# apache/arrow

Hardware: AMD Instinct MI355X
Metric: filter_take_mrows_per_s (higher is better)
Workload: dtype int64; 1 GPU; Filter+Take int64[1000000000] + validity (10% null), boolean mask 10% true, FilterOptions::DROP; take indices = the mask's row numbers (monotonic; indices_nonzero: uint64 through CallFunction, GetTakeIndices: uint32 in the mirror), no boundscheck; inputs = splitmix64 streams of SURVEY.md 8(d) (seeds 1,2,3); rows=1000000000, selected_rows=99992053, parallelism=single-gpu

## Files before the change

### arrow_amd/csrc/selection.hip

```cpp
#include "arx_common.h"

#include <string.h>

#include <algorithm>
#include <type_traits>

namespace arx {

struct FilterWsHeader {
  int64_t total;
  int64_t ntiles;
  int64_t ngroups;
  int64_t length;
  int64_t valid;
  int64_t pad[3];
};
static_assert(sizeof(FilterWsHeader) == 64, "header is one 64-byte line");

struct FilterWsView {
  FilterWsHeader* hdr;
  int64_t* group_excl;
  int64_t* group_total;
  uint32_t* tile_counts;
  int64_t* group_valid;
};

static inline int64_t num_tiles(int64_t length) { return ceil_div(length, kTileRows); }
static inline int64_t num_groups(int64_t length) {
  return ceil_div(num_tiles(length), kTilesPerGroup);
}

static inline FilterWsView ws_view(void* ws, int64_t length) {
  FilterWsView v;
  const int64_t ng = num_groups(length);
  uint8_t* p = static_cast<uint8_t*>(ws);
  v.hdr = reinterpret_cast<FilterWsHeader*>(p);
  v.group_excl = reinterpret_cast<int64_t*>(p + 64);
  v.group_total = v.group_excl + ng;
  v.tile_counts = reinterpret_cast<uint32_t*>(v.group_total + ng);
  v.group_valid = reinterpret_cast<int64_t*>(v.tile_counts + ng * kTilesPerGroup);
  return v;
}

__device__ __forceinline__ uint64_t emit_word(const Bits& mask, const Bits& mvalid, int64_t w,
                                              bool emit_null, bool invert,
                                              uint64_t* mask_valid_out) {
  uint64_t m = load_word(mask, w);
  const uint64_t mv = load_word(mvalid, w);
  *mask_valid_out = mv;
  if (emit_null || invert) {
    const uint64_t in_range = load_word(Bits{nullptr, 0, mask.length, 0}, w);
    if (invert) m = ~m & in_range;
    if (emit_null) return (m | ~mv) & in_range;
  }
  return m & mv;
}

template <bool VALID>
__global__ __launch_bounds__(kBlock) void count_kernel(Bits mask, Bits mvalid, Bits vvalid, int emit_null,
                                                       int invert, int64_t ntiles,
                                                       uint32_t* tile_counts,
                                                       int64_t* group_total, int64_t* group_valid) {
  __shared__ uint32_t wave_sums[kWavesPerBlock];
  __shared__ uint32_t wave_valid[kWavesPerBlock];
  const int lane = lane_id();
  const int wave = threadIdx.x >> 6;
  const int64_t group = blockIdx.x;
  const int64_t t0 = group * kTilesPerGroup + wave * 16;
  uint32_t mine = 0;
  uint32_t kv = 0;
#pragma unroll 4
  for (int i = 0; i < 16; ++i) {
    const int64_t t = t0 + i;
    uint32_t k = 0;
    if (t < ntiles) {
      uint64_t mv;
      const uint64_t e = emit_word(mask, mvalid, t * 64 + lane, emit_null != 0, invert != 0, &mv);
      k = __popcll(e);
      if constexpr (VALID) kv += __popcll(e & mv & load_word(vvalid, t * 64 + lane));
    }
    const uint32_t s = wave_reduce_sum_u32(k);
    if (lane == i) mine = s;
  }
  if (lane < 16) tile_counts[t0 + lane] = mine;
  const uint32_t wsum = wave_reduce_sum_u32(lane < 16 ? mine : 0u);
  if (lane == 0) wave_sums[wave] = wsum;
  if constexpr (VALID) {
    const uint32_t vsum = wave_reduce_sum_u32(kv);
    if (lane == 0) wave_valid[wave] = vsum;
  }
  __syncthreads();
  if (threadIdx.x == 0) {
    int64_t s = 0, v = 0;
    for (int i = 0; i < kWavesPerBlock; ++i) {
      s += wave_sums[i];
      if constexpr (VALID) v += wave_valid[i];
    }
    group_total[group] = s;
    if constexpr (VALID) group_valid[group] = v;
  }
}

__global__ __launch_bounds__(1024) void scan_kernel(const int64_t* group_total, int64_t ngroups,
                                                    int64_t* group_excl, FilterWsHeader* hdr,
                                                    const int64_t* group_valid = nullptr) {
  __shared__ int64_t wave_tot[16];
  __shared__ int64_t carry_s;
  __shared__ unsigned long long valid_s;
  const int tid = threadIdx.x;
  const int lane = tid & 63;
  const int wave = tid >> 6;
  if (tid == 0) carry_s = 0;
  if (tid == 0) valid_s = 0;
  __syncthreads();
  if (group_valid != nullptr) {
    int64_t mine = 0;
    for (int64_t i = tid; i < ngroups; i += 1024) mine += group_valid[i];
#pragma unroll
    for (int d = 32; d >= 1; d >>= 1) mine += __shfl_xor(mine, d, 64);
    if (lane == 0 && mine != 0) atomicAdd(&valid_s, static_cast<unsigned long long>(mine));
    __syncthreads();
  }
  for (int64_t base = 0; base < ngroups; base += 1024) {
    const int64_t i = base + tid;
    const int64_t v = i < ngroups ? group_total[i] : 0;
    int64_t x = v;
#pragma unroll
    for (int d = 1; d < 64; d <<= 1) {
      const int64_t n = __shfl_up(x, d, 64);
      if (lane >= d) x += n;
    }
    if (lane == 63) wave_tot[wave] = x;
    __syncthreads();
    int64_t wave_prefix = 0;
    for (int k = 0; k < wave; ++k) wave_prefix += wave_tot[k];
    const int64_t carry = carry_s;
    if (i < ngroups) group_excl[i] = carry + wave_prefix + x - v;
    __syncthreads();
    if (tid == 1023) carry_s = carry + wave_prefix + x;
    __syncthreads();
  }
  if (tid == 0) {
    hdr->total = carry_s;
    hdr->valid = static_cast<int64_t>(valid_s);
  }
}

struct CompactArgs {
  const uint8_t* values;
  Bits mask;
  Bits mvalid;
  Bits vvalid;
  int64_t length;
  int64_t ntiles;
  const uint32_t* tile_counts;
  const int64_t* group_excl;
  uint8_t* out_data;
  uint64_t* out_validity;
  int emit_null;
  int invert;
  int values_aligned16;
};

constexpr int kFlushBytes = 2048;

template <int RING>
struct __attribute__((aligned(16))) CompactLds {
  uint8_t ring[kWavesPerBlock][RING];
  uint64_t vbits[kWavesPerBlock][72];
};

template <int W>
struct ElemT;
template <> struct ElemT<1> { using type = uint8_t; };
template <> struct ElemT<2> { using type = uint16_t; };
template <> struct ElemT<4> { using type = uint32_t; };
template <> struct ElemT<8> { using type = uint64_t; };
template <> struct ElemT<16> { using type = uint4; };
struct Elem32 { uint4 lo, hi; };
template <> struct ElemT<32> { using type = Elem32; };

template <int W>
__device__ __forceinline__ typename ElemT<W>::type zero_elem() {
  if constexpr (W == 32) {
    return Elem32{make_uint4(0, 0, 0, 0), make_uint4(0, 0, 0, 0)};
  } else if constexpr (W == 16) {
    return make_uint4(0, 0, 0, 0);
  } else {
    return 0;
  }
}

constexpr int kSelNt = 3;

template <int W>
__device__ __forceinline__ typename ElemT<W>::type sel_load(const typename ElemT<W>::type* p, bool nt) {
  using E = typename ElemT<W>::type;
  if constexpr (W == 32) {
    return *p;
  } else if constexpr (W == 16) {
    return nt ? nt_load16(p) : *p;
  } else {
    return nt ? nt_load<E>(p) : *p;
  }
}
template <int W>
__device__ __forceinline__ void sel_store(typename ElemT<W>::type* p, typename ElemT<W>::type v) {
  using E = typename ElemT<W>::type;
  if constexpr (W == 32) {
    *p = v;
  } else if constexpr (W == 16) {
    if constexpr ((kSelNt & 2) != 0) nt_store16(p, v); else *p = v;
  } else {
    if constexpr ((kSelNt & 2) != 0) nt_store<E>(p, v); else *p = v;
  }
}

__device__ __forceinline__ void wave_lds_sync() {
  __builtin_amdgcn_fence(__ATOMIC_RELEASE, "wavefront");
  __builtin_amdgcn_wave_barrier();
  __builtin_amdgcn_fence(__ATOMIC_ACQUIRE, "wavefront");
}

template <int W, int RING>
__device__ __forceinline__ void flush_region(const uint8_t* ring, uint8_t* gbase, int64_t F,
                                             int64_t lo, int64_t hi, int lane) {
  using E = typename ElemT<W>::type;
  constexpr int R = 16 / W;
  const int ring_off = static_cast<int>(F & (RING - 1));
#pragma unroll
  for (int h = 0; h < kFlushBytes / (16 * kWave); ++h) {
    const int g = h * kWave + lane;
    const int64_t gs = F + g * 16;
    const int64_t ge = gs + 16;
    if (ge <= lo || gs >= hi) continue;
    const uint8_t* src = ring + ring_off + g * 16;
    uint8_t* dst = gbase + gs;
    if (gs >= lo && ge <= hi) {
      sel_store<16>(reinterpret_cast<uint4*>(dst), *reinterpret_cast<const uint4*>(src));
    } else {
#pragma unroll
      for (int e = 0; e < R; ++e) {
        const int64_t es = gs + e * W;
        if (es >= lo && es + W <= hi) {
          *reinterpret_cast<E*>(dst + e * W) = *reinterpret_cast<const E*>(src + e * W);
        }
      }
    }
  }
}

template <int W, int B>
struct Batch {
  using E = typename ElemT<W>::type;
  static constexpr int R = 16 / W;
  uint32_t bits[B];
  uint32_t zbits[B];
  uint32_t rank[B];
  E v[B][R];
};

template <int R, bool EMIT>
__device__ __forceinline__ void select_words(uint64_t Ew, uint32_t p, uint64_t Zw,
                                             int widx_base, int lane, uint64_t* wE, uint32_t* wp,
                                             uint64_t* wZ) {
  constexpr int kLanesPerWord = 64 / R;
  const int q_mine = lane / kLanesPerWord;
  uint64_t e = 0, z = 0;
  uint32_t pp = 0;
#pragma unroll
  for (int q = 0; q < R; ++q) {
    const int src = widx_base + q;
    const uint32_t lo = __builtin_amdgcn_readlane(static_cast<uint32_t>(Ew), src);
    const uint32_t hi = __builtin_amdgcn_readlane(static_cast<uint32_t>(Ew >> 32), src);
    const uint32_t pq = __builtin_amdgcn_readlane(p, src);
    uint64_t zq = 0;
    if constexpr (EMIT) {
      const uint32_t zlo = __builtin_amdgcn_readlane(static_cast<uint32_t>(Zw), src);
      const uint32_t zhi = __builtin_amdgcn_readlane(static_cast<uint32_t>(Zw >> 32), src);
      zq = (static_cast<uint64_t>(zhi) << 32) | zlo;
    }
    if (q == q_mine) {
      e = (static_cast<uint64_t>(hi) << 32) | lo;
      pp = pq;
      z = zq;
    }
  }
  *wE = e;
  *wp = pp;
  *wZ = z;
}

struct TileCtx {
  uint64_t Ew, Zw;
  uint32_t p;
  int lane;
  int64_t tile_row0;
  const uint8_t* values;
  __amdgpu_buffer_rsrc_t rsrc;
};

template <int W, bool IOTA, bool EMIT, bool ALIGNED, int B>
__device__ __forceinline__ void issue_batch(const TileCtx& c, int j0, Batch<W, B>& b) {
  using E = typename ElemT<W>::type;
  constexpr int R = 16 / W;
  constexpr int kRowsPerIter = kWave * R;
#pragma unroll
  for (int i = 0; i < B; ++i) {
    const int j = j0 + i;
    const int row_in_tile = j * kRowsPerIter + c.lane * R;
    const int bpos = row_in_tile & 63;
    uint64_t wE, wZ;
    uint32_t wp;
    select_words<R, EMIT>(c.Ew, c.p, c.Zw, j * R, c.lane, &wE, &wp, &wZ);
    b.bits[i] = static_cast<uint32_t>(wE >> bpos) & ((1u << R) - 1u);
    b.zbits[i] = static_cast<uint32_t>(wZ >> bpos) & ((1u << R) - 1u);
    b.rank[i] = wp + __popcll(wE & low_mask64(bpos));
    if constexpr (IOTA) {
#pragma unroll
      for (int r = 0; r < R; ++r) b.v[i][r] = static_cast<E>(c.tile_row0 + row_in_tile + r);
    } else {
      const int64_t row = c.tile_row0 + row_in_tile;
      const uint8_t* src = c.values + row * static_cast<int64_t>(W);
      if constexpr (ALIGNED) {
        const uint32_t voff = b.bits[i] != 0 ? static_cast<uint32_t>(row_in_tile * W) : kBufferSkip;
        const uint4 q = (kSelNt & 1) ? buffer_load_b128_nt(c.rsrc, voff) : buffer_load_b128(c.rsrc, voff);
        if constexpr (W == 16) {
          b.v[i][0] = q;
        } else {
          const E* qe = reinterpret_cast<const E*>(&q);
#pragma unroll
          for (int r = 0; r < R; ++r) b.v[i][r] = qe[r];
        }
      } else {
#pragma unroll
        for (int r = 0; r < R; ++r) {
          b.v[i][r] = zero_elem<W>();
          if ((b.bits[i] >> r) & 1u) {
            if constexpr (W == 16) {
              const uint64_t* s64 = reinterpret_cast<const uint64_t*>(src + r * W);
              const uint64_t lo64 = s64[0], hi64 = s64[1];
              b.v[i][r] = make_uint4(static_cast<uint32_t>(lo64), static_cast<uint32_t>(lo64 >> 32),
                                     static_cast<uint32_t>(hi64), static_cast<uint32_t>(hi64 >> 32));
            } else {
              b.v[i][r] = *reinterpret_cast<const E*>(src + r * W);
            }
          }
        }
      }
    }
  }
}

template <int W, int B, int RING>
__device__ __forceinline__ void consume_batch(const Batch<W, B>& b, uint8_t* ring, int64_t a0) {
  using E = typename ElemT<W>::type;
  constexpr int R = 16 / W;
#pragma unroll
  for (int i = 0; i < B; ++i) {
    if (b.bits[i] != 0) {
      uint32_t rk = b.rank[i];
#pragma unroll
      for (int r = 0; r < R; ++r) {
        if ((b.bits[i] >> r) & 1u) {
          E e = b.v[i][r];
          if ((b.zbits[i] >> r) & 1u) e = zero_elem<W>();
          const int ro = static_cast<int>((a0 + static_cast<int64_t>(rk) * W) & (RING - 1));
          *reinterpret_cast<E*>(ring + ro) = e;
          ++rk;
        }
      }
    }
  }
}

template <int W, bool IOTA, bool EMIT, bool ALIGNED, int B, bool PIPE>
__global__ __launch_bounds__(kBlock) void compact_kernel(CompactArgs a) {
  using E = typename ElemT<W>::type;
  constexpr int R = 16 / W;
  constexpr int kRowsPerIter = kWave * R;
  constexpr int kIters = kTileRows / kRowsPerIter;
  constexpr int kWordsPerIter = kRowsPerIter / 64;
  constexpr int kBatches = kIters / B;
  constexpr int RING = (B <= 2) ? 4096 : 8192;
  static_assert(kIters % B == 0, "batch must divide the iteration count");
  static_assert(!PIPE || kBatches % 2 == 0, "pipelined form walks the batches in pairs");

  __shared__ CompactLds<RING> lds;

  const int lane = lane_id();
  const int wave = __builtin_amdgcn_readfirstlane(threadIdx.x >> 6);
  const int64_t t = static_cast<int64_t>(blockIdx.x) * kWavesPerBlock + wave;
  if (t >= a.ntiles) return;

  const int64_t w = t * 64 + lane;
  uint64_t mv;
  const uint64_t Ew = emit_word(a.mask, a.mvalid, w, EMIT, a.invert != 0, &mv);
  const uint32_t k = __popcll(Ew);
  const uint32_t incl = wave_inclusive_scan_u32(k);
  const uint32_t p = incl - k;
  const uint32_t total = __shfl(incl, 63, 64);
  if (total == 0) return;

  const int64_t grp = t >> 6;
  const int tin = static_cast<int>(t & 63);
  const uint32_t cprev = lane < tin ? a.tile_counts[grp * kTilesPerGroup + lane] : 0u;
  const int64_t off = a.group_excl[grp] + wave_reduce_sum_u32(cprev);

  uint8_t* ring = lds.ring[wave];
  const int64_t a0 =
      static_cast<int64_t>((reinterpret_cast<uint64_t>(a.out_data) + static_cast<uint64_t>(off) * W) &
                           (kFlushBytes - 1));
  uint8_t* gbase = a.out_data + (off * static_cast<int64_t>(W) - a0);
  int64_t flushed = 0;

  TileCtx c;
  c.Ew = Ew;
  c.Zw = EMIT ? (Ew & ~mv) : 0;
  c.p = p;
  c.lane = lane;
  c.tile_row0 = t * kTileRows;
  c.values = a.values;
  c.rsrc = make_rsrc(IOTA ? nullptr : a.values + c.tile_row0 * static_cast<int64_t>(W),
                     static_cast<uint32_t>(kTileRows * W));

  auto flush_check = [&](int next_batch) {
    const uint32_t cum = next_batch < kBatches
                             ? __builtin_amdgcn_readlane(p, next_batch * B * kWordsPerIter)
                             : total;
    const int64_t written = a0 + static_cast<int64_t>(cum) * W;
    if (written - flushed >= kFlushBytes) {
      wave_lds_sync();
      while (written - flushed >= kFlushBytes) {
        flush_region<W, RING>(ring, gbase, flushed, a0, written, lane);
        flushed += kFlushBytes;
      }
      wave_lds_sync();
    }
  };

  bool tile_done = false;
  if constexpr (IOTA) {
    if (a0 + static_cast<int64_t>(total) * W <= RING) {
      uint64_t m = Ew;
      uint32_t rk = p;
      while (m != 0) {
        const int bpos = __ffsll(static_cast<unsigned long long>(m)) - 1;
// ... 301 lines not shown
    const int64_t base = c * (64 * U);
    int64_t pos[U];
    uint64_t idx[U];
    bool ok[U];
#pragma unroll
    for (int u = 0; u < U; ++u) {
      const int64_t p = base + u * 64 + lane;
      pos[u] = p <= last ? p : last;
      idx[u] = static_cast<uint64_t>((kSelNt & 1) ? nt_load<IdxT>(indices + pos[u]) : indices[pos[u]]);
    }
#pragma unroll
    for (int u = 0; u < U; ++u) {
      ok[u] = (base + u * 64 + lane) <= last;
      if constexpr (HAS_IV) {
        const uint64_t wbits = load_word_nb(a.ivalid, (base >> 6) + u);
        ok[u] = ok[u] && ((wbits >> lane) & 1ull);
      }
    }
    E val[U];
#pragma unroll
    for (int u = 0; u < U; ++u) {
      const E* src = ok[u] ? (values + idx[u]) : (out + pos[u]);
      val[u] = sel_load<W>(src, (kSelNt & 4) != 0);
    }
    if constexpr (HAS_SV) {
      uint8_t vb[U];
#pragma unroll
      for (int u = 0; u < U; ++u) {
        const uint64_t bit = ok[u] ? static_cast<uint64_t>(a.src_valid_offset) + idx[u] : 0;
        vb[u] = a.src_valid_bytes[bit >> 3];
      }
#pragma unroll
      for (int u = 0; u < U; ++u) {
        const uint64_t bit = static_cast<uint64_t>(a.src_valid_offset) + idx[u];
        ok[u] = ok[u] && ((vb[u] >> (bit & 7)) & 1);
      }
    }
#pragma unroll
    for (int u = 0; u < U; ++u) {
      const int64_t p = base + u * 64 + lane;
      if (p <= last) sel_store<W>(out + p, ok[u] ? val[u] : zero_elem<W>());
      const uint64_t vbal = __ballot(ok[u]);
      nvalid += __popcll(vbal);
      if (a.out_validity != nullptr && lane == 0 && (base + u * 64) <= last) {
        a.out_validity[(base >> 6) + u] = vbal;
      }
    }
  }
  if (a.valid_count != nullptr && lane == 0 && nvalid != 0) atomicAdd(a.valid_count, nvalid);
}

template <int UB> struct RowUnit;
template <> struct RowUnit<1> { typedef uint8_t type; };
template <> struct RowUnit<2> { typedef uint16_t type; };
template <> struct RowUnit<4> { typedef uint32_t type; };
template <> struct RowUnit<8> { typedef uint64_t type; };
template <> struct RowUnit<16> { typedef arx_u32x4 type; };

template <int UB, typename IdxT, bool HAS_IV, bool HAS_SV>
__global__ __launch_bounds__(kBlock) void take_rows_kernel(TakeArgs a, uint32_t units_per_row) {
  using E = typename RowUnit<UB>::type;
  const int lane = lane_id();
  const int64_t nwaves = static_cast<int64_t>(gridDim.x) * kWavesPerBlock;
  const int64_t wave_g = static_cast<int64_t>(blockIdx.x) * kWavesPerBlock + __builtin_amdgcn_readfirstlane(threadIdx.x >> 6);
  const int64_t nchunks = (a.length + 63) >> 6;
  const int64_t last = a.length - 1;
  const IdxT* __restrict__ indices = reinterpret_cast<const IdxT*>(a.indices);
  const E* __restrict__ values = reinterpret_cast<const E*>(a.values);
  E* __restrict__ out = reinterpret_cast<E*>(a.out_data);
  uint64_t nvalid = 0;
  for (int64_t c = wave_g; c < nchunks; c += nwaves) {
    const int64_t base = c << 6;
    const int64_t p = base + lane <= last ? base + lane : last;
    uint64_t idx = static_cast<uint64_t>(indices[p]);
    bool ok = base + lane <= last;
    if constexpr (HAS_IV) ok = ok && ((load_word_nb(a.ivalid, base >> 6) >> lane) & 1ull);
    if constexpr (HAS_SV) {
      const uint64_t bit = ok ? static_cast<uint64_t>(a.src_valid_offset) + idx : 0;
      ok = ok && ((a.src_valid_bytes[bit >> 3] >> (bit & 7)) & 1);
    }
    if (!ok) idx = 0;
    const uint64_t vbal = __ballot(ok);
    nvalid += __popcll(vbal);
    if (a.out_validity != nullptr && lane == 0) a.out_validity[base >> 6] = vbal;
    const int rows_here = static_cast<int>(last - base + 1 < 64 ? last - base + 1 : 64);
    const uint32_t total = static_cast<uint32_t>(rows_here) * units_per_row;
    const uint32_t idx_lo = static_cast<uint32_t>(idx), idx_hi = static_cast<uint32_t>(idx >> 32);
    for (uint32_t t = lane; t < ((total + 63u) & ~63u); t += 64) {
      const uint32_t tt = t < total ? t : total - 1;
      const uint32_t row = tt / units_per_row;
      const uint32_t j = tt - row * units_per_row;
      const uint64_t src = (static_cast<uint64_t>(__shfl(idx_hi, static_cast<int>(row), 64)) << 32) | __shfl(idx_lo, static_cast<int>(row), 64);
      const bool row_ok = (vbal >> row) & 1ull;
      E v = E{};
      if (row_ok) v = values[src * units_per_row + j];
      if (t < total) out[(static_cast<uint64_t>(base) + row) * units_per_row + j] = v;
    }
  }
  if (a.valid_count != nullptr && lane == 0 && nvalid != 0) atomicAdd(a.valid_count, nvalid);
}

constexpr int kTakeMaxCols = 16;
struct TakeColsArgs {
  const uint8_t* values[kTakeMaxCols];
  const uint8_t* src_valid_bytes[kTakeMaxCols];
  int64_t src_valid_offset[kTakeMaxCols];
  uint8_t* out_data[kTakeMaxCols];
  uint64_t* out_validity[kTakeMaxCols];
  int width[kTakeMaxCols];
  int num_cols;
  const uint8_t* indices;
  Bits ivalid;
  int64_t length;
  unsigned long long* valid_counts;
};

template <int W, int U>
__device__ __forceinline__ uint64_t take_one_column(const TakeColsArgs& a, int c, const int64_t (&pos)[U],
                                                    const uint64_t (&idx)[U], const bool (&ok0)[U], int64_t base,
                                                    int64_t last, int lane) {
  using E = typename ElemT<W>::type;
  const E* __restrict__ values = reinterpret_cast<const E*>(a.values[c]);
  E* __restrict__ out = reinterpret_cast<E*>(a.out_data[c]);
  const uint8_t* __restrict__ svb = a.src_valid_bytes[c];
  const uint64_t svo = static_cast<uint64_t>(a.src_valid_offset[c]);
  E val[U];
  bool ok[U];
#pragma unroll
  for (int u = 0; u < U; ++u) {
    const E* src = ok0[u] ? (values + idx[u]) : (out + pos[u]);
    val[u] = *src;
    ok[u] = ok0[u];
  }
  if (svb != nullptr) {
    uint8_t vb[U];
#pragma unroll
    for (int u = 0; u < U; ++u) vb[u] = svb[(ok0[u] ? svo + idx[u] : 0) >> 3];
#pragma unroll
    for (int u = 0; u < U; ++u) ok[u] = ok[u] && ((vb[u] >> ((svo + idx[u]) & 7)) & 1);
  }
  uint64_t nvalid = 0;
#pragma unroll
  for (int u = 0; u < U; ++u) {
    const int64_t p = base + u * 64 + lane;
    if (p <= last) out[p] = ok[u] ? val[u] : zero_elem<W>();
    const uint64_t vbal = __ballot(ok[u]);
    nvalid += __popcll(vbal);
    if (a.out_validity[c] != nullptr && lane == 0 && (base + u * 64) <= last) a.out_validity[c][(base >> 6) + u] = vbal;
  }
  return nvalid;
}

template <typename IdxT, bool HAS_IV>
__global__ __launch_bounds__(kBlock) void take_columns_kernel(TakeColsArgs a) {
  constexpr int U = 4;
  const int lane = lane_id();
  const int64_t nwaves = static_cast<int64_t>(gridDim.x) * kWavesPerBlock;
  const int64_t wave_g = static_cast<int64_t>(blockIdx.x) * kWavesPerBlock +
                         __builtin_amdgcn_readfirstlane(threadIdx.x >> 6);
  const int64_t nchunks = (a.length + 64 * U - 1) / (64 * U);
  const int64_t last = a.length - 1;
  const IdxT* __restrict__ indices = reinterpret_cast<const IdxT*>(a.indices);
  uint64_t nvalid[kTakeMaxCols];
  for (int c = 0; c < kTakeMaxCols; ++c) nvalid[c] = 0;
  for (int64_t ch = wave_g; ch < nchunks; ch += nwaves) {
    const int64_t base = ch * (64 * U);
    int64_t pos[U];
    uint64_t idx[U];
    bool ok0[U];
#pragma unroll
    for (int u = 0; u < U; ++u) {
      const int64_t p = base + u * 64 + lane;
      pos[u] = p <= last ? p : last;
      idx[u] = static_cast<uint64_t>(indices[pos[u]]);
    }
#pragma unroll
    for (int u = 0; u < U; ++u) {
      ok0[u] = (base + u * 64 + lane) <= last;
      if constexpr (HAS_IV) {
        const uint64_t wbits = load_word_nb(a.ivalid, (base >> 6) + u);
        ok0[u] = ok0[u] && ((wbits >> lane) & 1ull);
      }
    }
    for (int c = 0; c < a.num_cols; ++c) {
      uint64_t nv;
      switch (a.width[c]) {
        case 1: nv = take_one_column<1, U>(a, c, pos, idx, ok0, base, last, lane); break;
        case 2: nv = take_one_column<2, U>(a, c, pos, idx, ok0, base, last, lane); break;
        case 4: nv = take_one_column<4, U>(a, c, pos, idx, ok0, base, last, lane); break;
        case 8: nv = take_one_column<8, U>(a, c, pos, idx, ok0, base, last, lane); break;
        case 16: nv = take_one_column<16, U>(a, c, pos, idx, ok0, base, last, lane); break;
        default: nv = take_one_column<32, U>(a, c, pos, idx, ok0, base, last, lane); break;
      }
      nvalid[c] += nv;
    }
  }
  if (a.valid_counts != nullptr && lane == 0) {
    for (int c = 0; c < a.num_cols; ++c) {
      if (nvalid[c] != 0) atomicAdd(a.valid_counts + c, nvalid[c]);
    }
  }
}

template <typename IdxT>
__global__ __launch_bounds__(kBlock) void take_bits_kernel(TakeArgs a, int64_t value_bit_offset) {
  const int lane = lane_id();
  const int64_t nwaves = static_cast<int64_t>(gridDim.x) * kWavesPerBlock;
  const int64_t wave_g = static_cast<int64_t>(blockIdx.x) * kWavesPerBlock +
                         __builtin_amdgcn_readfirstlane(threadIdx.x >> 6);
  const int64_t nwords = (a.length + 63) >> 6;
  const int64_t last = a.length - 1;
  const IdxT* __restrict__ indices = reinterpret_cast<const IdxT*>(a.indices);
  uint64_t* __restrict__ out = reinterpret_cast<uint64_t*>(a.out_data);
  uint64_t nvalid = 0;
  for (int64_t w = wave_g; w < nwords; w += nwaves) {
    const int64_t p = (w << 6) + lane;
    const int64_t pc = p <= last ? p : last;
    const uint64_t idx = static_cast<uint64_t>(indices[pc]);
    bool ok = p <= last && ((load_word(a.ivalid, w) >> lane) & 1ull);
    if (ok && a.src_valid_bytes != nullptr) {
      const uint64_t vb = static_cast<uint64_t>(a.src_valid_offset) + idx;
      ok = (a.src_valid_bytes[vb >> 3] >> (vb & 7)) & 1;
    }
    bool bit = false;
    if (ok) {
      const uint64_t b = static_cast<uint64_t>(value_bit_offset) + idx;
      bit = (a.values[b >> 3] >> (b & 7)) & 1;
    }
    const uint64_t data_bal = __ballot(bit);
    const uint64_t valid_bal = __ballot(ok);
    nvalid += __popcll(valid_bal);
    if (lane == 0) {
      out[w] = data_bal;
      if (a.out_validity != nullptr) a.out_validity[w] = valid_bal;
    }
  }
  if (a.valid_count != nullptr && lane == 0 && nvalid != 0) atomicAdd(a.valid_count, nvalid);
}

struct BoundsWs {
  unsigned long long first_bad_pos;
  long long bad_value_signed;
  unsigned long long bad_value_unsigned;
  int64_t pad[5];
};

template <typename IdxT>
__global__ __launch_bounds__(kBlock) void bounds_kernel(const uint8_t* indices, Bits ivalid,
                                                        int64_t length, uint64_t upper,
                                                        BoundsWs* ws) {
  const int64_t stride = static_cast<int64_t>(gridDim.x) * blockDim.x;
  unsigned long long bad = ~0ull;
  for (int64_t i = static_cast<int64_t>(blockIdx.x) * blockDim.x + threadIdx.x; i < length;
       i += stride) {
    const IdxT v = reinterpret_cast<const IdxT*>(indices)[i];
    const bool valid = (load_word(ivalid, i >> 6) >> (i & 63)) & 1ull;
    bool oob;
    if constexpr (std::is_signed<IdxT>::value) {
      oob = v < 0 || static_cast<uint64_t>(v) >= upper;
    } else {
      oob = static_cast<uint64_t>(v) >= upper;
    }
    if (valid && oob) {
      bad = static_cast<unsigned long long>(i);
      break;
    }
  }
  if (bad != ~0ull) atomicMin(&ws->first_bad_pos, bad);
}

template <typename IdxT>
__global__ void bounds_fetch_kernel(const uint8_t* indices, BoundsWs* ws) {
  const unsigned long long pos = ws->first_bad_pos;
  if (pos == ~0ull) return;
  const IdxT v = reinterpret_cast<const IdxT*>(indices)[pos];
  ws->bad_value_signed = static_cast<long long>(v);
  ws->bad_value_unsigned = static_cast<unsigned long long>(v);
}

static int check_mask(const ArxSpan* mask, int null_selection) {
  if (mask == nullptr) {
    set_error("filter mask is NULL");
    return ARX_INVALID;
  }
  if (mask->length < 0 || mask->offset < 0) {
    set_error("negative length/offset");
    return ARX_INVALID;
  }
  if (mask->length > 0 && mask->data == nullptr) {
    set_error("filter mask has no data buffer");
    return ARX_INVALID;
  }
  if (null_selection != ARX_FILTER_DROP && null_selection != ARX_FILTER_EMIT_NULL) {
    set_error("bad null_selection %d", null_selection);
    return ARX_INVALID;
  }
  return ARX_OK;
}

static inline const void* effective_validity(const ArxSpan* s) {
  return (s->null_count != 0) ? s->validity : nullptr;
}

static int launch_count(const ArxSpan* mask, int null_selection, void* ws, size_t ws_bytes,
                        hipStream_t st, int invert = 0, const ArxSpan* values = nullptr) {
  const int rc = check_mask(mask, null_selection);
  if (rc != ARX_OK) return rc;
  const size_t need = arx_filter_workspace_bytes(mask->length);
  if (ws == nullptr || ws_bytes < need) {
    set_error("filter workspace too small: %zu < %zu", ws_bytes, need);
    return ARX_INVALID;
  }
  if ((reinterpret_cast<uint64_t>(ws) & 63) != 0) {
    set_error("filter workspace must be 64-byte aligned");
    return ARX_INVALID;
  }
  FilterWsView v = ws_view(ws, mask->length);
  const int64_t nt = num_tiles(mask->length);
  const int64_t ng = num_groups(mask->length);
  FilterWsHeader h{};
  h.total = 0;
  h.ntiles = nt;
  h.ngroups = ng;
  h.length = mask->length;
  ARX_HIP(hipMemcpyAsync(v.hdr, &h, sizeof(h), hipMemcpyHostToDevice, st));
  if (mask->length == 0) return ARX_OK;
  const Bits mb = make_bits(mask->data, mask->offset, mask->length);
  const Bits mvb = make_bits(effective_validity(mask), mask->offset, mask->length);
  if (values != nullptr) {
    const Bits vvb = make_bits(effective_validity(values), values->offset, mask->length);
    hipLaunchKernelGGL((count_kernel<true>), dim3(static_cast<unsigned>(ng)), dim3(kBlock), 0, st, mb, mvb, vvb,
                       null_selection, invert, nt, v.tile_counts, v.group_total, v.group_valid);
    ARX_CHECK_LAUNCH("count_kernel");
    hipLaunchKernelGGL(scan_kernel, dim3(1), dim3(1024), 0, st, v.group_total, ng, v.group_excl, v.hdr,
                       static_cast<const int64_t*>(v.group_valid));
  } else {
    hipLaunchKernelGGL((count_kernel<false>), dim3(static_cast<unsigned>(ng)), dim3(kBlock), 0, st, mb, mvb, mvb,
                       null_selection, invert, nt, v.tile_counts, v.group_total, static_cast<int64_t*>(nullptr));
    ARX_CHECK_LAUNCH("count_kernel");
    hipLaunchKernelGGL(scan_kernel, dim3(1), dim3(1024), 0, st, v.group_total, ng, v.group_excl, v.hdr,
                       static_cast<const int64_t*>(nullptr));
  }
  ARX_CHECK_LAUNCH("scan_kernel");
  return ARX_OK;
}

static Knob<int> g_filter_batch{4};
static Knob<int> g_filter_pipe{1};
static Knob<int> g_filter_sparse{-1};

template <int W, bool IOTA, bool EMIT, bool ALIGNED>
static void launch_compact_e(const CompactArgs& a, unsigned grid, hipStream_t st) {
  constexpr int kIters = kTileRows / (kWave * (16 / W));
  constexpr int kBig = kIters >= 8 ? 4 : 2;
  if (ALIGNED && g_filter_batch >= 4 && g_filter_pipe) {
    hipLaunchKernelGGL((compact_kernel<W, IOTA, EMIT, ALIGNED, kBig, true>), dim3(grid),
                       dim3(kBlock), 0, st, a);
  } else {
    hipLaunchKernelGGL((compact_kernel<W, IOTA, EMIT, ALIGNED, 1, false>), dim3(grid), dim3(kBlock),
                       0, st, a);
  }
}

template <int W, bool IOTA>
static void launch_compact_w(const CompactArgs& a, unsigned grid, hipStream_t st) {
  const bool aligned = IOTA || a.values_aligned16 != 0;
  if (a.emit_null) {
    if (aligned) launch_compact_e<W, IOTA, true, true>(a, grid, st);
    else if constexpr (!IOTA) launch_compact_e<W, IOTA, true, false>(a, grid, st);
  } else {
    if (aligned) launch_compact_e<W, IOTA, false, true>(a, grid, st);
    else if constexpr (!IOTA) launch_compact_e<W, IOTA, false, false>(a, grid, st);
  }
}

template <int W, bool IOTA = false>
static void launch_sparse_w(const CompactArgs& a, unsigned grid, hipStream_t st) {
  if (a.emit_null) {
    hipLaunchKernelGGL((compact_sparse_kernel<W, true, IOTA>), dim3(grid), dim3(kBlock), 0, st, a);
  } else {
    hipLaunchKernelGGL((compact_sparse_kernel<W, false, IOTA>), dim3(grid), dim3(kBlock), 0, st, a);
  }
}

static int launch_compact(bool iota, int W, const CompactArgs& a, hipStream_t st,
                          int64_t out_length = -1) {
  const unsigned grid = static_cast<unsigned>(ceil_div(a.ntiles, kWavesPerBlock));
  const bool sparse = !iota && !a.invert &&
                      (g_filter_sparse == 1 ||
                       (g_filter_sparse < 0 &&
                        (W >= 8 || (out_length >= 0 && out_length * 4 <= a.length))));
  if (iota && !a.invert && g_filter_sparse != 0 && (W == 2 || W == 4 || W == 8)) {
    if (W == 2) launch_sparse_w<2, true>(a, grid, st);
    else if (W == 4) launch_sparse_w<4, true>(a, grid, st);
    else launch_sparse_w<8, true>(a, grid, st);
    ARX_CHECK_LAUNCH("compact_sparse_kernel<IOTA>");
    return ARX_OK;
  }
  if (sparse) {
    switch (W) {
      case 1: launch_sparse_w<1>(a, grid, st); break;
      case 2: launch_sparse_w<2>(a, grid, st); break;
      case 4: launch_sparse_w<4>(a, grid, st); break;
      case 8: launch_sparse_w<8>(a, grid, st); break;
      case 16: launch_sparse_w<16>(a, grid, st); break;
      case 32: launch_sparse_w<32>(a, grid, st); break;
      default:
        set_error("unsupported byte width %d for the gfx950 filter", W);
        return ARX_NOT_IMPLEMENTED;
    }
    ARX_CHECK_LAUNCH("compact_sparse_kernel");
    return ARX_OK;
  }
  if (iota) {
    switch (W) {
      case 2: launch_compact_w<2, true>(a, grid, st); break;
      case 4: launch_compact_w<4, true>(a, grid, st); break;
      default:
        set_error("unsupported index width %d", W);
        return ARX_NOT_IMPLEMENTED;
    }
  } else {
    switch (W) {
      case 1: launch_compact_w<1, false>(a, grid, st); break;
      case 2: launch_compact_w<2, false>(a, grid, st); break;
      case 4: launch_compact_w<4, false>(a, grid, st); break;
      case 8: launch_compact_w<8, false>(a, grid, st); break;
      case 16: launch_compact_w<16, false>(a, grid, st); break;
      default:
        set_error("unsupported byte width %d for the gfx950 filter", W);
        return ARX_NOT_IMPLEMENTED;
    }
  }
  ARX_CHECK_LAUNCH("compact_kernel");
  return ARX_OK;
}

int set_selection_option(const char* name, int64_t value) {
  if (strcmp(name, "filter_batch") == 0) {
    g_filter_batch = value >= 4 ? 4 : 1;
    return 1;
  }
  if (strcmp(name, "filter_pipe") == 0) {
    g_filter_pipe = value != 0;
    return 1;
  }
  if (strcmp(name, "filter_sparse") == 0) {
    g_filter_sparse = value < 0 ? -1 : (value != 0);
    return 1;
  }
  return 0;
}

static int zero_out_validity(void* out_validity, int64_t out_length, hipStream_t st) {
  if (out_validity == nullptr) return ARX_OK;
  if ((reinterpret_cast<uint64_t>(out_validity) & 7) != 0) {
    set_error("out_validity must be 8-byte aligned");
    return ARX_INVALID;
  }
  if (out_length < 0) {
    set_error("out_length (from arx_filter_count) is required when out_validity is given");
    return ARX_INVALID;
  }
  if (out_length > 0) {
    ARX_HIP(hipMemsetAsync(out_validity, 0, static_cast<size_t>(ceil_div(out_length, 64)) * 8, st));
  }
  return ARX_OK;
}

size_t selection_workspace_bytes(int64_t length) { return arx_filter_workspace_bytes(length); }

int selection_bit_positions(const void* bitmap, int64_t bit_offset, int64_t length, bool invert,
                            void* ws, size_t ws_bytes, uint32_t* out, int64_t* out_count_host,
                            hipStream_t st) {
  ArxSpan m{};
  m.validity = nullptr;
  m.data = bitmap;
  m.offset = bit_offset;
  m.length = length;
  m.null_count = 0;
  int rc = launch_count(&m, ARX_FILTER_DROP, ws, ws_bytes, st, invert ? 1 : 0);
  if (rc != ARX_OK) return rc;
  int64_t total = 0;
  ARX_HIP(hipMemcpyAsync(&total, ws, sizeof(int64_t), hipMemcpyDeviceToHost, st));
  ARX_HIP(hipStreamSynchronize(st));
  *out_count_host = total;
  if (total == 0) return ARX_OK;
  FilterWsView v = ws_view(ws, length);
  CompactArgs a{};
  a.values = nullptr;
  a.mask = make_bits(bitmap, bit_offset, length);
  a.mvalid = make_bits(nullptr, 0, length);
  a.vvalid = make_bits(nullptr, 0, length);
  a.length = length;
  a.ntiles = num_tiles(length);
  a.tile_counts = v.tile_counts;
  a.group_excl = v.group_excl;
  a.out_data = reinterpret_cast<uint8_t*>(out);
  a.out_validity = nullptr;
  a.emit_null = 0;
  a.invert = invert ? 1 : 0;
  a.values_aligned16 = 1;
  return launch_compact(true, 4, a, st);
}

}

using namespace arx;

extern "C" {

size_t arx_filter_workspace_bytes(int64_t length) {
  if (length < 0) length = 0;
  const int64_t ng = num_groups(length);
  return static_cast<size_t>(64 + ng * 16 + ng * kTilesPerGroup * 4 + ng * 8 + 64);
}

int arx_filter_count_async(const ArxSpan* mask, int null_selection, void* ws, size_t ws_bytes,
                           void* stream) {
  return launch_count(mask, null_selection, ws, ws_bytes, as_stream(stream));
}

int arx_filter_count_nulls(const ArxSpan* values, const ArxSpan* mask, int null_selection, void* ws, size_t ws_bytes,
                           int64_t* out_length, int64_t* out_null_count, void* stream) {
  if (out_length == nullptr || out_null_count == nullptr || values == nullptr) {
    set_error("values / out_length / out_null_count is NULL");
    return ARX_INVALID;
  }
  if (mask != nullptr && values->length != mask->length) {
    set_error("filter values and mask differ in length (%lld vs %lld)", static_cast<long long>(values->length),
              static_cast<long long>(mask->length));
    return ARX_INVALID;
  }
  hipStream_t st = as_stream(stream);
  const int rc = launch_count(mask, null_selection, ws, ws_bytes, st, 0, values);
  if (rc != ARX_OK) return rc;
  int64_t hdr[5] = {0, 0, 0, 0, 0};
  ARX_HIP(hipMemcpyAsync(hdr, ws, sizeof(hdr), hipMemcpyDeviceToHost, st));
  ARX_HIP(hipStreamSynchronize(st));
  *out_length = hdr[0];
  *out_null_count = mask->length == 0 ? 0 : hdr[0] - hdr[4];
  return ARX_OK;
}

int arx_filter_count(const ArxSpan* mask, int null_selection, void* ws, size_t ws_bytes,
                     int64_t* out_length, void* stream) {
  if (out_length == nullptr) {
    set_error("out_length is NULL");
    return ARX_INVALID;
  }
  hipStream_t st = as_stream(stream);
  const int rc = launch_count(mask, null_selection, ws, ws_bytes, st);
  if (rc != ARX_OK) return rc;
  int64_t total = 0;
  ARX_HIP(hipMemcpyAsync(&total, ws, sizeof(int64_t), hipMemcpyDeviceToHost, st));
  ARX_HIP(hipStreamSynchronize(st));
  *out_length = total;
  return ARX_OK;
}

int arx_filter_exec(const ArxSpan* values, int byte_width, const ArxSpan* mask, int null_selection,
                    const void* ws, int64_t out_length, void* out_data, void* out_validity,
                    void* stream) {
  int rc = check_mask(mask, null_selection);
  if (rc != ARX_OK) return rc;
  if (values == nullptr || ws == nullptr) {
    set_error("values/ws is NULL");
    return ARX_INVALID;
  }
  if (values->length != mask->length) {
    set_error("Array arguments must all be the same length (values %lld vs filter %lld)",
              static_cast<long long>(values->length), static_cast<long long>(mask->length));
    return ARX_INVALID;
  }
  if (mask->length == 0) return ARX_OK;
  if (values->data == nullptr || out_data == nullptr) {
    set_error("values/out data buffer is NULL");
    return ARX_INVALID;
  }
  hipStream_t st = as_stream(stream);
  FilterWsView v = ws_view(const_cast<void*>(ws), mask->length);
  CompactArgs a{};
  a.values = static_cast<const uint8_t*>(values->data) + values->offset * byte_width;
  a.mask = make_bits(mask->data, mask->offset, mask->length);
  a.mvalid = make_bits(effective_validity(mask), mask->offset, mask->length);
  a.vvalid = make_bits(effective_validity(values), values->offset, values->length);
  a.length = mask->length;
  a.ntiles = num_tiles(mask->length);
  a.tile_counts = v.tile_counts;
  a.group_excl = v.group_excl;
  a.out_data = static_cast<uint8_t*>(out_data);
  a.out_validity = static_cast<uint64_t*>(out_validity);
  a.emit_null = null_selection == ARX_FILTER_EMIT_NULL && a.mvalid.base != nullptr;
  a.values_aligned16 = (reinterpret_cast<uint64_t>(a.values) & 15) == 0;
  if ((reinterpret_cast<uint64_t>(out_data) % byte_width) != 0) {
    set_error("out_data is not aligned to the element width");
    return ARX_INVALID;
  }
  rc = zero_out_validity(out_validity, out_length, st);
  if (rc != ARX_OK) return rc;
  return launch_compact(false, byte_width, a, st, out_length);
}

int arx_expand_by_mask(const void* dense, int byte_width, const ArxSpan* mask, const void* ws, void* out_data,
                       void* stream) {
  int rc = check_mask(mask, ARX_FILTER_DROP);
  if (rc != ARX_OK) return rc;
  if (ws == nullptr) {
    set_error("ws is NULL (run arx_filter_count on the mask first)");
    return ARX_INVALID;
  }
  if (mask->length == 0) return ARX_OK;
  if (out_data == nullptr || (reinterpret_cast<uint64_t>(out_data) % byte_width) != 0 ||
      (dense != nullptr && (reinterpret_cast<uint64_t>(dense) % byte_width) != 0)) {
    set_error("expand: NULL or misaligned buffer");
    return ARX_INVALID;
  }
  FilterWsView v = ws_view(const_cast<void*>(ws), mask->length);
  CompactArgs a{};
  a.values = static_cast<const uint8_t*>(dense);
  a.mask = make_bits(mask->data, mask->offset, mask->length);
  a.mvalid = make_bits(effective_validity(mask), mask->offset, mask->length);
  a.length = mask->length;
  a.ntiles = num_tiles(mask->length);
  a.tile_counts = v.tile_counts;
  a.group_excl = v.group_excl;
  a.out_data = static_cast<uint8_t*>(out_data);
  const unsigned grid = static_cast<unsigned>(ceil_div(a.ntiles, kWavesPerBlock));
  hipStream_t st = as_stream(stream);
  switch (byte_width) {
    case 1: hipLaunchKernelGGL((expand_kernel<1>), dim3(grid), dim3(kBlock), 0, st, a); break;
    case 2: hipLaunchKernelGGL((expand_kernel<2>), dim3(grid), dim3(kBlock), 0, st, a); break;
    case 4: hipLaunchKernelGGL((expand_kernel<4>), dim3(grid), dim3(kBlock), 0, st, a); break;
    case 8: hipLaunchKernelGGL((expand_kernel<8>), dim3(grid), dim3(kBlock), 0, st, a); break;
    case 16: hipLaunchKernelGGL((expand_kernel<16>), dim3(grid), dim3(kBlock), 0, st, a); break;
    default:
      set_error("unsupported byte width %d for expand", byte_width);
      return ARX_NOT_IMPLEMENTED;
  }
  ARX_CHECK_LAUNCH("expand_kernel");
  return ARX_OK;
}

int arx_mask_to_indices(const ArxSpan* mask, int null_selection, const void* ws, int64_t out_length,
                        int index_width, void* out_indices, void* out_validity, void* stream) {
  int rc = check_mask(mask, null_selection);
  if (rc != ARX_OK) return rc;
  if (ws == nullptr) {
    set_error("ws is NULL");
    return ARX_INVALID;
  }
  if (index_width != 2 && index_width != 4 && index_width != 8) {
    set_error("index_width must be 2, 4 or 8");
    return ARX_INVALID;
  }
  if (index_width == 8 && (g_filter_sparse == 0 || null_selection == ARX_FILTER_EMIT_NULL)) {
    set_error("index_width 8 is served by the gather form with DROP only");
    return ARX_NOT_IMPLEMENTED;
  }
  if (mask->length > static_cast<int64_t>(UINT32_MAX)) {
    set_error("Filter length exceeds UINT32_MAX, consider a different strategy for selecting elements");
    return ARX_NOT_IMPLEMENTED;
  }
  if (index_width == 2 && mask->length > 65535) {
    set_error("index_width 2 requires length <= 65535");
    return ARX_INVALID;
  }
  if (mask->length == 0) return ARX_OK;
  if (out_indices == nullptr) {
    set_error("out_indices is NULL");
    return ARX_INVALID;
  }
  hipStream_t st = as_stream(stream);
  FilterWsView v = ws_view(const_cast<void*>(ws), mask->length);
  CompactArgs a{};
  a.values = nullptr;
  a.mask = make_bits(mask->data, mask->offset, mask->length);
  a.mvalid = make_bits(effective_validity(mask), mask->offset, mask->length);
  a.vvalid = make_bits(nullptr, 0, mask->length);
  a.length = mask->length;
  a.ntiles = num_tiles(mask->length);
  a.tile_counts = v.tile_counts;
  a.group_excl = v.group_excl;
  a.out_data = static_cast<uint8_t*>(out_indices);
  a.out_validity = static_cast<uint64_t*>(out_validity);
  a.emit_null = null_selection == ARX_FILTER_EMIT_NULL && a.mvalid.base != nullptr;
  a.values_aligned16 = 1;
  const bool emit = a.emit_null != 0;
  if (emit && out_validity == nullptr) {
    set_error("EMIT_NULL with a nullable mask needs out_validity");
    return ARX_INVALID;
  }
  rc = zero_out_validity(out_validity, out_length, st);
  if (rc != ARX_OK) return rc;
  return launch_compact(true, index_width, a, st);
}

size_t arx_take_workspace_bytes(void) { return sizeof(BoundsWs); }

int arx_check_index_bounds(const ArxSpan* indices, int index_type, uint64_t upper_limit, void* ws,
                           size_t ws_bytes, void* stream) {
  if (indices == nullptr || ws == nullptr || ws_bytes < sizeof(BoundsWs)) {
    set_error("bad arguments to arx_check_index_bounds");
    return ARX_INVALID;
  }
  if (indices->length == 0) return ARX_OK;
  hipStream_t st = as_stream(stream);
  static const int widths[8] = {1, 1, 2, 2, 4, 4, 8, 8};
  if (index_type < 0 || index_type > 7) {
    set_error("Invalid index type for boundschecking");
    return ARX_INVALID;
  }
  const int iw = widths[index_type];
  const uint8_t* idx = static_cast<const uint8_t*>(indices->data) + indices->offset * iw;
  const Bits iv = make_bits(effective_validity(indices), indices->offset, indices->length);
  BoundsWs* bws = static_cast<BoundsWs*>(ws);
  BoundsWs init{};
  init.first_bad_pos = ~0ull;
  ARX_HIP(hipMemcpyAsync(bws, &init, sizeof(init), hipMemcpyHostToDevice, st));
  const int64_t blocks = std::min<int64_t>(ceil_div(indices->length, kBlock), 256 * 8);
  const dim3 grid(static_cast<unsigned>(blocks)), block(kBlock);
#define ARX_BOUNDS(T)                                                                        \
  hipLaunchKernelGGL((bounds_kernel<T>), grid, block, 0, st, idx, iv, indices->length,       \
                     upper_limit, bws);                                                      \
  hipLaunchKernelGGL((bounds_fetch_kernel<T>), dim3(1), dim3(1), 0, st, idx, bws)
  switch (index_type) {
    case ARX_UINT8: ARX_BOUNDS(uint8_t); break;
    case ARX_INT8: ARX_BOUNDS(int8_t); break;
    case ARX_UINT16: ARX_BOUNDS(uint16_t); break;
    case ARX_INT16: ARX_BOUNDS(int16_t); break;
    case ARX_UINT32: ARX_BOUNDS(uint32_t); break;
    case ARX_INT32: ARX_BOUNDS(int32_t); break;
    case ARX_UINT64: ARX_BOUNDS(uint64_t); break;
    default: ARX_BOUNDS(int64_t); break;
  }
#undef ARX_BOUNDS
  ARX_CHECK_LAUNCH("bounds_kernel");
  BoundsWs res{};
  ARX_HIP(hipMemcpyAsync(&res, bws, sizeof(res), hipMemcpyDeviceToHost, st));
  ARX_HIP(hipStreamSynchronize(st));
  if (res.first_bad_pos != ~0ull) {
    const bool is_signed = (index_type & 1) != 0;
    if (is_signed) {
      set_error("Index %lld out of bounds", res.bad_value_signed);
    } else {
      set_error("Index %llu out of bounds", res.bad_value_unsigned);
    }
// ... 295 lines not shown
```

Measured before the change: 305,800 Mrows/s.

## Fuse filter count and group scan into one last-block-scans kernel

Replaces the separate count kernel and single-block scan kernel with one kernel. Each block writes its group totals and takes an atomic ticket, and the last block to finish performs the exclusive scan over group totals and writes the header. This removes one kernel launch and the serial gap between the two, at the cost of a ticket counter in the header, reliance on correct memory ordering, and a tail where one block scans alone. The fused path is on by default behind a knob.

After: 306,400 Mrows/s, median of 6. Within noise of the previous version (+0.2%).

```diff
diff --git a/arrow_amd/csrc/selection.hip b/arrow_amd/csrc/selection.hip
--- a/arrow_amd/csrc/selection.hip
+++ b/arrow_amd/csrc/selection.hip
@@ -13,7 +13,9 @@
   int64_t ngroups;
   int64_t length;
   int64_t valid;
-  int64_t pad[3];
+  uint32_t ticket;
+  uint32_t pad0;
+  int64_t pad[2];
 };
 static_assert(sizeof(FilterWsHeader) == 64, "header is one 64-byte line");
 
@@ -143,6 +145,154 @@
   if (tid == 0) {
     hdr->total = carry_s;
     hdr->valid = static_cast<int64_t>(valid_s);
+  }
+}
+
+constexpr int kScanPerThread = 16;
+
+template <bool HAS>
+__device__ __forceinline__ void count_words(const Bits& b, int64_t w0, int lane, uint64_t (&out)[16]) {
+  if constexpr (!HAS) {
+#pragma unroll
+    for (int i = 0; i < 16; ++i) out[i] = ~uint64_t(0);
+  } else {
+    const int64_t last = b.nphys - 1;
+    if (b.shift == 0) {
+#pragma unroll
+      for (int i = 0; i < 16; ++i) {
+        const int64_t w = w0 + i * 64 + lane;
+        out[i] = b.base[w < last ? w : last];
+      }
+    } else {
+      uint64_t hi[16];
+#pragma unroll
+      for (int i = 0; i < 16; ++i) {
+        const int64_t w = w0 + i * 64 + lane;
+        out[i] = b.base[w < last ? w : last];
+        hi[i] = b.base[(w + 1) < last ? (w + 1) : last];
+      }
+#pragma unroll
+      for (int i = 0; i < 16; ++i) out[i] = (out[i] >> b.shift) | ((hi[i] << 1) << (63 - b.shift));
+    }
+  }
+}
+
+__device__ __forceinline__ uint64_t in_range_word(int64_t length, int64_t w) {
+  const int64_t remain = length - (w << 6);
+  return remain >= 64 ? ~uint64_t(0) : (remain <= 0 ? uint64_t(0) : ((uint64_t(1) << remain) - 1));
+}
+
+template <bool VALID, bool HAS_MV, bool HAS_VV>
+__global__ __launch_bounds__(kBlock) void count_scan_kernel(Bits mask, Bits mvalid, Bits vvalid, int emit_null,
+                                                            int invert, int64_t ngroups, FilterWsView v) {
+  __shared__ uint32_t wave_sums[kWavesPerBlock];
+  __shared__ uint32_t wave_valid[kWavesPerBlock];
+  __shared__ int64_t scan_tot[kWavesPerBlock];
+  __shared__ int64_t scan_valid[kWavesPerBlock];
+  __shared__ uint32_t is_last;
+  const int lane = lane_id();
+  const int wave = threadIdx.x >> 6;
+  const int64_t group = blockIdx.x;
+  const int64_t t0 = group * kTilesPerGroup + wave * 16;
+  const int64_t w0 = t0 * 64;
+
+  uint64_t m[16], mv[16], vv[16];
+  count_words<true>(mask, w0, lane, m);
+  count_words<HAS_MV>(mvalid, w0, lane, mv);
+  count_words<VALID && HAS_VV>(vvalid, w0, lane, vv);
+
+  uint32_t pk[8];
+  uint32_t kv = 0;
+#pragma unroll
+  for (int i = 0; i < 16; ++i) {
+    const uint64_t in_range = in_range_word(mask.length, w0 + i * 64 + lane);
+    const uint64_t mvw = mv[i] & in_range;
+    uint64_t e = m[i] & in_range;
+    if (invert) e = ~e & in_range;
+    e = emit_null ? (e | (~mvw & in_range)) : (e & mvw);
+    const uint32_t k = __popcll(e);
+    if constexpr (VALID) kv += __popcll(e & mvw & vv[i]);
+    if ((i & 1) == 0) pk[i >> 1] = k; else pk[i >> 1] |= k << 16;
+  }
+  uint32_t mine = 0;
+#pragma unroll
+  for (int j = 0; j < 8; ++j) {
+    const uint32_t s = wave_reduce_sum_u32(pk[j]);
+    if ((lane >> 1) == j) mine = (lane & 1) ? (s >> 16) : (s & 0xffffu);
+  }
+  if (lane < 16) v.tile_counts[t0 + lane] = mine;
+  const uint32_t wsum = wave_reduce_sum_u32(lane < 16 ? mine : 0u);
+  if (lane == 0) wave_sums[wave] = wsum;
+  if constexpr (VALID) {
+    const uint32_t vsum = wave_reduce_sum_u32(kv);
+    if (lane == 0) wave_valid[wave] = vsum;
+  }
+  __syncthreads();
+  if (threadIdx.x == 0) {
+    int64_t s = 0, vs = 0;
+    for (int i = 0; i < kWavesPerBlock; ++i) {
+      s += wave_sums[i];
+      if constexpr (VALID) vs += wave_valid[i];
+    }
+    __hip_atomic_store(&v.group_total[group], s, __ATOMIC_RELAXED, __HIP_MEMORY_SCOPE_AGENT);
+    if constexpr (VALID) __hip_atomic_store(&v.group_valid[group], vs, __ATOMIC_RELAXED, __HIP_MEMORY_SCOPE_AGENT);
+#if defined(__HIP_DEVICE_COMPILE__)
+    __builtin_amdgcn_s_waitcnt(0);
+#endif
+    is_last = atomicAdd(&v.hdr->ticket, 1u) == gridDim.x - 1 ? 1u : 0u;
+  }
+  __syncthreads();
+  if (is_last == 0) return;
+  __threadfence();
+
+  const int tid = threadIdx.x;
+  int64_t carry = 0, valid_mine = 0;
+  for (int64_t base = 0; base < ngroups; base += kBlock * kScanPerThread) {
+    const int64_t g0 = base + static_cast<int64_t>(tid) * kScanPerThread;
+    int64_t x[kScanPerThread];
+#pragma unroll
+    for (int j = 0; j < kScanPerThread; ++j) {
+      const int64_t g = (g0 + j) < ngroups ? (g0 + j) : (ngroups - 1);
+      x[j] = __hip_atomic_load(&v.group_total[g], __ATOMIC_RELAXED, __HIP_MEMORY_SCOPE_AGENT);
+      if ((g0 + j) >= ngroups) x[j] = 0;
+      if constexpr (VALID) {
+        const int64_t gv = __hip_atomic_load(&v.group_valid[g], __ATOMIC_RELAXED, __HIP_MEMORY_SCOPE_AGENT);
+        valid_mine += (g0 + j) < ngroups ? gv : 0;
+      }
+    }
+    int64_t sum = 0;
+#pragma unroll
+    for (int j = 0; j < kScanPerThread; ++j) sum += x[j];
+    const int64_t incl = static_cast<int64_t>(wave_inclusive_scan_u64(static_cast<uint64_t>(sum)));
+    if (lane == 63) scan_tot[wave] = incl;
+    __syncthreads();
+    int64_t before = carry + incl - sum;
+    int64_t pass_total = 0;
+    for (int k = 0; k < kWavesPerBlock; ++k) {
+      if (k < wave) before += scan_tot[k];
+      pass_total += scan_tot[k];
+    }
+#pragma unroll
+    for (int j = 0; j < kScanPerThread; ++j) {
+      if ((g0 + j) < ngroups) v.group_excl[g0 + j] = before;
+      before += x[j];
+    }
+    carry += pass_total;
+    __syncthreads();
+  }
+  if constexpr (VALID) {
+    const int64_t vsum = static_cast<int64_t>(wave_reduce_sum_u64(static_cast<uint64_t>(valid_mine)));
+    if (lane == 0) scan_valid[wave] = vsum;
+    __syncthreads();
+  }
+  if (tid == 0) {
+    int64_t valid = 0;
+    if constexpr (VALID) {
+      for (int k = 0; k < kWavesPerBlock; ++k) valid += scan_valid[k];
+    }
+    v.hdr->total = carry;
+    v.hdr->valid = valid;
+    v.hdr->ticket = 0;
   }
 }
 
@@ -1050,6 +1200,8 @@
   return (s->null_count != 0) ? s->validity : nullptr;
 }
 
+static Knob<int> g_filter_count_fused{1};
+
 static int launch_count(const ArxSpan* mask, int null_selection, void* ws, size_t ws_bytes,
                         hipStream_t st, int invert = 0, const ArxSpan* values = nullptr) {
   const int rc = check_mask(mask, null_selection);
@@ -1075,6 +1227,24 @@
   if (mask->length == 0) return ARX_OK;
   const Bits mb = make_bits(mask->data, mask->offset, mask->length);
   const Bits mvb = make_bits(effective_validity(mask), mask->offset, mask->length);
+  if (g_filter_count_fused) {
+    const Bits vvb = make_bits(values != nullptr ? effective_validity(values) : nullptr, values != nullptr ? values->offset : 0,
+                               mask->length);
+    const dim3 grid(static_cast<unsigned>(ng)), block(kBlock);
+    const bool has_mv = mvb.base != nullptr, has_vv = vvb.base != nullptr;
+#define ARX_COUNT_SCAN(VALID, MV, VV) \
+  hipLaunchKernelGGL((count_scan_kernel<VALID, MV, VV>), grid, block, 0, st, mb, mvb, vvb, null_selection, invert, ng, v)
+    if (values == nullptr) {
+      if (has_mv) ARX_COUNT_SCAN(false, true, false); else ARX_COUNT_SCAN(false, false, false);
+    } else if (has_mv) {
+      if (has_vv) ARX_COUNT_SCAN(true, true, true); else ARX_COUNT_SCAN(true, true, false);
+    } else {
+      if (has_vv) ARX_COUNT_SCAN(true, false, true); else ARX_COUNT_SCAN(true, false, false);
+    }
+#undef ARX_COUNT_SCAN
+    ARX_CHECK_LAUNCH("count_scan_kernel");
+    return ARX_OK;
+  }
   if (values != nullptr) {
     const Bits vvb = make_bits(effective_validity(values), values->offset, mask->length);
     hipLaunchKernelGGL((count_kernel<true>), dim3(static_cast<unsigned>(ng)), dim3(kBlock), 0, st, mb, mvb, vvb,
@@ -1191,6 +1361,10 @@
   }
   if (strcmp(name, "filter_pipe") == 0) {
     g_filter_pipe = value != 0;
+    return 1;
+  }
+  if (strcmp(name, "filter_count_fused") == 0) {
+    g_filter_count_fused = value != 0;
     return 1;
   }
   if (strcmp(name, "filter_sparse") == 0) {
```
